# evergreen-ci/evergreen

Hardware: NVIDIA H100
Metric: tasks scheduled/sec over N distros; host-allocator decisions/sec at 1/2/4/8 GPU (higher is better)
Workload: dtype int64

## Files before the change

evergreen_b200/csrc/evg_plan_general.cuh:

```cuda
#pragma once

#ifndef EVG_OCC_GLINK
#define EVG_OCC_GLINK 4
#endif
#ifndef EVG_OCC_GALLOC
#define EVG_OCC_GALLOC 4
#endif
#ifndef EVG_OCC_GFILL
#define EVG_OCC_GFILL 4
#endif
#ifndef EVG_OCC_GUNIT
#define EVG_OCC_GUNIT 4
#endif
#ifndef EVG_OCC_GBEST
#define EVG_OCC_GBEST 4
#endif
#ifndef EVG_GTASK_OCC
#define EVG_GTASK_OCC 2
#endif
constexpr int kGTile = 2048;

struct DGen {
  int64_t n_tiles;
  int64_t tile0;
  const int32_t* tile_distro;
  const int64_t* tile_start;
  const int64_t* dtile_off;
  unsigned long long* vmm;
  uint32_t* key_lo[2];
  uint32_t* key_hi[2];
  uint32_t* idx[2];
  uint32_t* e;
  uint32_t* tile_sum;
  uint32_t* tile_hist;
  uint4* wl;
  struct URec* pay;
  unsigned int* ccount;
  uint4* tie;
  int32_t* maxpass;
  uint32_t* run;
  uint32_t* pown;
  uint32_t* pver;
  uint32_t* pedge;
  uint32_t* sedge;
  uint32_t* rank;
  unsigned int* rcount;
  uint2* blist;
  unsigned int* bcount;
  uint4* usum;
  uint2* hlist;
  unsigned int* hcount;
  int64_t* tv;
};

__device__ __forceinline__ int gen_bits(const DGen& G, int d) {
  const unsigned long long r = G.vmm[2 * d] - G.vmm[2 * d + 1];
  return r == 0 ? 0 : 64 - __clzll((long long)r);
}
__device__ __forceinline__ int gen_npass(int bits) { return (bits + 7) >> 3; }

struct __align__(16) URec {
  int32_t prio, nd;
  int64_t exp_ns, qb;
  int32_t tgo;
  uint32_t lif;
};
static_assert(sizeof(URec) == 32, "one L2 sector per member");
constexpr uint32_t kRecGrouped = 1u << 22, kRecWaitOver = 1u << 23;
constexpr uint32_t kRunOwn = 1u << 31, kRunEntry = kRunOwn - 1u;
__device__ __forceinline__ uint32_t rec_li(const URec& r) { return r.lif & 0x1FFFFFu; }
__device__ __forceinline__ URec rec_load(const URec* p) {
  const uint4 a = reinterpret_cast<const uint4*>(p)[0], b = reinterpret_cast<const uint4*>(p)[1];
  URec r;
  r.prio = int32_t(a.x); r.nd = int32_t(a.y); r.exp_ns = int64_t((unsigned long long)a.z | ((unsigned long long)a.w << 32));
  r.qb = int64_t((unsigned long long)b.x | ((unsigned long long)b.y << 32)); r.tgo = int32_t(b.z); r.lif = b.w;
  return r;
}
__device__ __forceinline__ void rec_store(URec* p, const URec& r) {
  reinterpret_cast<uint4*>(p)[0] = make_uint4(uint32_t(r.prio), uint32_t(r.nd), uint32_t(uint64_t(r.exp_ns)), uint32_t(uint64_t(r.exp_ns) >> 32));
  reinterpret_cast<uint4*>(p)[1] = make_uint4(uint32_t(uint64_t(r.qb)), uint32_t(uint64_t(r.qb) >> 32), uint32_t(r.tgo), r.lif);
}

__global__ void k_ginit(DGen G, const int32_t* __restrict__ general_list, int n) {
  const int k = blockIdx.x * blockDim.x + threadIdx.x;
  if (k == 0) { *G.ccount = 0u; *G.maxpass = 0; *G.rcount = 0u; *G.hcount = 0u; *G.bcount = 0u; }
  if (k >= n) return;
  const int d = general_list[k];
  G.vmm[2 * d] = 0ull;
  G.vmm[2 * d + 1] = ~0ull;
}

__global__ void __launch_bounds__(256) k_gmark(DTasks T, DDistros D, DWork W, DGen G) {
  if (*W.err) return;
  const int tile = int(blockIdx.x + G.tile0);
  const int d = G.tile_distro[tile];
  const int64_t base = D.task_off[d], end = D.task_off[d + 1];
  const int64_t lo = max(G.tile_start[tile], base), hi = min(G.tile_start[tile] + kGTile, end);
  for (int64_t t = lo + threadIdx.x; t < hi; t += 256)
    for (int64_t e = T.dep_off[t]; e < T.dep_off[t + 1]; e++) W.has_dep[base + T.dep_idx[e]] = 1;
}

struct TileFold {
  unsigned int c[10];
  unsigned long long s[4];
// ... 478 lines not shown
      }
      if (lane == 0) {
        if (hi > __ldcg(G.vmm + 2 * d0)) atomicMax(G.vmm + 2 * d0, hi);
        if (lo < __ldcg(G.vmm + 2 * d0 + 1)) atomicMin(G.vmm + 2 * d0 + 1, lo);
      }
    } else if (d >= 0) {
      if (kk > __ldcg(G.vmm + 2 * d)) atomicMax(G.vmm + 2 * d, kk);
      if (kk < __ldcg(G.vmm + 2 * d + 1)) atomicMin(G.vmm + 2 * d + 1, kk);
    }
  }
}

__global__ void k_gsched(DGen G, const int32_t* __restrict__ general_list, int n) {
  const int k = blockIdx.x * blockDim.x + threadIdx.x;
  if (k >= n) return;
  const int np = gen_npass(gen_bits(G, general_list[k]));
  if (np > 0) atomicMax(G.maxpass, np);
}

__global__ void __launch_bounds__(256) k_gsum(DDistros D, DGen G) {
  const int tile = int(blockIdx.x + G.tile0);
  const int d = G.tile_distro[tile];
  const int64_t base = D.task_off[d], end = D.task_off[d + 1];
  const int64_t lo = max(G.tile_start[tile], base), hi = min(G.tile_start[tile] + kGTile, end);
  uint32_t sum = 0;
  for (int64_t t = lo + threadIdx.x; t < hi; t += 256) sum += G.e[t];
  sum = __reduce_add_sync(0xffffffffu, sum);
  __shared__ uint32_t sw[8];
  if ((threadIdx.x & 31) == 0) sw[threadIdx.x >> 5] = sum;
  __syncthreads();
  if (threadIdx.x == 0) G.tile_sum[tile] = sw[0] + sw[1] + sw[2] + sw[3] + sw[4] + sw[5] + sw[6] + sw[7];
}
// ... 32 lines not shown

__device__ __forceinline__ void gen_put(const DGen& G, int64_t base, uint32_t pos, unsigned long long vmax_ord, bool wide,
                                        int64_t v, uint32_t li) {
  const unsigned long long key = vmax_ord - ord_i64(v);
  G.key_lo[0][base + pos] = uint32_t(key);
  if (wide) G.key_hi[0][base + pos] = uint32_t(key >> 32);
  G.idx[0][base + pos] = li;
}

__global__ void __launch_bounds__(256) k_gplace(DDistros D, DWork W, DGen G, int use_e) {
  const int tile = int(blockIdx.x + G.tile0);
  const int d = G.tile_distro[tile];
  const int64_t base = D.task_off[d], end = D.task_off[d + 1];
  const int64_t ts = G.tile_start[tile];
  const unsigned long long vmax_ord = G.vmm[2 * d];
  const bool wide = gen_bits(G, d) > 32;
  const int tid = threadIdx.x, lane = tid & 31, warp = tid >> 5;
  const int64_t t8 = ts + 8 * int64_t(tid);
  const bool interior = t8 >= base && t8 + 7 < end;
  uint32_t ev[8];
  uint32_t sum = 0;
  if (use_e) {
    if (interior) {
      const uint4 a = *reinterpret_cast<const uint4*>(G.e + t8), b = *reinterpret_cast<const uint4*>(G.e + t8 + 4);
      ev[0] = a.x; ev[1] = a.y; ev[2] = a.z; ev[3] = a.w; ev[4] = b.x; ev[5] = b.y; ev[6] = b.z; ev[7] = b.w;
    } else {
#pragma unroll
      for (int m = 0; m < 8; m++) { const int64_t t = t8 + m; ev[m] = (t >= base && t < end) ? G.e[t] : 0u; }
    }
#pragma unroll
    for (int m = 0; m < 8; m++) sum += ev[m];
// ... 20 lines not shown
      vv[m] = x.x; vv[m + 1] = x.y;
    }
    if (use_e) {
      const uint32_t h0 = *reinterpret_cast<const uint32_t*>(W.has_dep + t8), h1 = *reinterpret_cast<const uint32_t*>(W.has_dep + t8 + 4);
#pragma unroll
      for (int m = 0; m < 4; m++) dsp |= (((h0 >> (8 * m + 1)) & 1u) << m) | (((h1 >> (8 * m + 1)) & 1u) << (m + 4));
    }
  } else {
#pragma unroll
    for (int m = 0; m < 8; m++) {
      const int64_t t = t8 + m;
      const bool in = t >= base && t < end;
      vv[m] = in ? G.tv[t] : 0;
      if (use_e && in && (W.has_dep[t] & 2)) dsp |= 1u << m;
    }
  }
  if (use_e) {
    constexpr int kStage = 3072;
    __shared__ uint32_t st_lo[kStage], st_ix[kStage], st_hi[kStage];
    __shared__ uint32_t s_total;
    const uint32_t p_tile = G.tile_sum[tile];
    if (tid == 255) s_total = run + sum - p_tile;
    uint32_t ps[8];
#pragma unroll
    for (int m = 0; m < 8; m++) { ps[m] = run; run += ev[m]; }
    if (interior) {
      *reinterpret_cast<uint4*>(G.e + t8) = make_uint4(ps[0], ps[1], ps[2], ps[3]);
      *reinterpret_cast<uint4*>(G.e + t8 + 4) = make_uint4(ps[4], ps[5], ps[6], ps[7]);
    } else {
#pragma unroll
// ... 64 lines not shown
  uint32_t pos = G.e[base + a];
  const uint32_t cnt = W.unit_n[slot];
  if (cnt <= 64) {
    pos += __popcll(W.unit_mask[slot] & ((1ull << myrk) - 1ull));
  } else {
    const uint32_t* run = G.run + W.head[slot];
    for (uint32_t i = 0; i < cnt; i++) {
      const uint4 tq = G.tie[run[i] & kRunEntry];
      if (tq.z == slot && tq.y < myrk) pos++;
    }
  }
  gen_put(G, base, pos, G.vmm[2 * d], gen_bits(G, d) > 32, G.tv[t], uint32_t(int64_t(t) - base));
  }
}

__device__ __forceinline__ bool gen_tile(const DDistros& D, const DGen& G, int tile, int j, int* d_out, int64_t* seg, int64_t* lo,
                                         int* cnt, bool* wide) {
  const int d = G.tile_distro[tile];
  const int bits = gen_bits(G, d);
  if (j >= gen_npass(bits)) return false;
  const int64_t base = D.task_off[d], end = D.task_off[d + 1];
  const int64_t a = max(G.tile_start[tile], base), b = min(G.tile_start[tile] + kGTile, end);
  *d_out = d; *seg = base; *lo = a; *cnt = int(b - a); *wide = bits > 32;
  return true;
}

__global__ void __launch_bounds__(256) k_ghist(int j, DDistros D, DGen G) {
  if (j >= *G.maxpass) return;
  int d, cnt; int64_t seg, lo; bool wide;
  const int tile = int(blockIdx.x + G.tile0);
  if (!gen_tile(D, G, tile, j, &d, &seg, &lo, &cnt, &wide)) return;
  const uint32_t* src = (j < 4 ? G.key_lo[j & 1] : G.key_hi[j & 1]) + lo;
  const int shift = 8 * (j & 3);
  __shared__ uint32_t h[256];
  h[threadIdx.x] = 0;
  __syncthreads();
  for (int i = threadIdx.x; i < cnt; i += 256) atomicAdd(&h[(src[i] >> shift) & 255u], 1u);
  __syncthreads();
  G.tile_hist[int64_t(tile) * 256 + threadIdx.x] = h[threadIdx.x];
}

__global__ void __launch_bounds__(1024) k_gdscan(int j, const int32_t* __restrict__ general_list, DGen G) {
  if (j >= *G.maxpass) return;
  const int d = general_list[blockIdx.x];
  if (j >= gen_npass(gen_bits(G, d))) return;
  const int dg = threadIdx.x & 255, grp = threadIdx.x >> 8;
  const int64_t t0 = G.dtile_off[d], nt = G.dtile_off[d + 1] - t0;
  const int64_t per = (nt + 3) / 4;
  const int64_t a = t0 + (grp * per < nt ? grp * per : nt), b = t0 + ((grp + 1) * per < nt ? (grp + 1) * per : nt);
  uint32_t* h = G.tile_hist + dg;
  uint32_t sum = 0;
  int64_t tile = a;
  for (; tile + 8 <= b; tile += 8) {
    uint32_t x[8];
#pragma unroll
    for (int k = 0; k < 8; k++) x[k] = h[(tile + k) * 256];
#pragma unroll
    for (int k = 0; k < 8; k++) sum += x[k];
  }
  for (; tile < b; tile++) sum += h[tile * 256];
  __shared__ uint32_t part[4][256];
  __shared__ uint32_t s[256];
  part[grp][dg] = sum;
  __syncthreads();
  const uint32_t total = part[0][dg] + part[1][dg] + part[2][dg] + part[3][dg];
  if (grp == 0) s[dg] = total;
  __syncthreads();
  for (int o = 1; o < 256; o <<= 1) {
    uint32_t v = 0;
    if (grp == 0 && dg >= o) v = s[dg - o];
    __syncthreads();
    if (grp == 0) s[dg] += v;
    __syncthreads();
  }
  uint32_t run = s[dg] - total;
  for (int g = 0; g < grp; g++) run += part[g][dg];
  tile = a;
  for (; tile + 8 <= b; tile += 8) {
    uint32_t x[8];
#pragma unroll
    for (int k = 0; k < 8; k++) x[k] = h[(tile + k) * 256];
#pragma unroll
    for (int k = 0; k < 8; k++) { h[(tile + k) * 256] = run; run += x[k]; }
  }
  for (; tile < b; tile++) { const uint32_t x = h[tile * 256]; h[tile * 256] = run; run += x; }
}

template <bool WIDE>
__device__ __forceinline__ void gscatter_tile(int j, const DGen& G, int tile, int64_t seg, int64_t lo, int cnt, uint32_t (*wcnt)[256],
                                              uint32_t* s_lo, uint32_t* s_ix, uint32_t* s_hi, int32_t* s_delta, uint32_t* s_wsum) {
  constexpr bool wide = WIDE;
  const int sb = j & 1, db = sb ^ 1;
  const int tid = threadIdx.x, warp = tid >> 5, lane = tid & 31;
#pragma unroll
  for (int w = 0; w < 8; w++) wcnt[w][tid] = 0u;
  __syncthreads();
  const unsigned lt = (1u << lane) - 1u;
  const int shift = 8 * (j & 3);
  const bool use_hi = j >= 4;
  const uint32_t* src_lo = G.key_lo[sb] + lo;
  const uint32_t* src_hi = G.key_hi[sb] + lo;
  const uint32_t* src_ix = G.idx[sb] + lo;
  uint32_t kl[8], kh[8], ix[8], dg[8], rk[8];
#pragma unroll
  for (int k = 0; k < 8; k++) {
    const int i = (warp * 8 + k) * 32 + lane;
    const bool ok = i < cnt;
    kl[k] = ok ? src_lo[i] : 0u;
    kh[k] = (ok && wide) ? src_hi[i] : 0u;
    ix[k] = ok ? src_ix[i] : 0u;
  }
  unsigned peers[8];
#pragma unroll
  for (int k = 0; k < 8; k++) {
    const int i = (warp * 8 + k) * 32 + lane;
    dg[k] = i < cnt ? (((use_hi ? kh[k] : kl[k]) >> shift) & 255u) : 256u;
    peers[k] = __match_any_sync(0xffffffffu, dg[k]);
  }
#pragma unroll
  for (int k = 0; k < 8; k++) {
    rk[k] = 0;
    if (dg[k] < 256u && (peers[k] & lt) == 0u) rk[k] = atomicAdd(&wcnt[warp][dg[k]], uint32_t(__popc(peers[k])));
  }
#pragma unroll
  for (int k = 0; k < 8; k++) rk[k] = __shfl_sync(0xffffffffu, rk[k], __ffs(peers[k]) - 1) + uint32_t(__popc(peers[k] & lt));
  __syncthreads();
  {
    uint32_t x[8], tot = 0;
#pragma unroll
    for (int w = 0; w < 8; w++) { x[w] = wcnt[w][tid]; tot += x[w]; }
    uint32_t inc = tot;
#pragma unroll
    for (int o = 1; o < 32; o <<= 1) { const uint32_t y = __shfl_up_sync(0xffffffffu, inc, o); if (lane >= o) inc += y; }
    if (lane == 31) s_wsum[warp] = inc;
    __syncthreads();
    uint32_t before = 0;
#pragma unroll
    for (int w = 0; w < 8; w++) before += w < warp ? s_wsum[w] : 0u;
    const uint32_t lbase = before + inc - tot;
    s_delta[tid] = int32_t(G.tile_hist[int64_t(tile) * 256 + tid]) - int32_t(lbase);
    uint32_t run = lbase;
#pragma unroll
    for (int w = 0; w < 8; w++) { wcnt[w][tid] = run; run += x[w]; }
  }
  __syncthreads();
#pragma unroll
  for (int k = 0; k < 8; k++) {
    if (dg[k] < 256u) {
      const uint32_t lp = wcnt[warp][dg[k]] + rk[k];
      s_lo[lp] = kl[k];
      s_ix[lp] = ix[k];
      if (wide) s_hi[lp] = kh[k];
    }
  }
  __syncthreads();
  uint32_t* dst_lo = G.key_lo[db] + seg;
  uint32_t* dst_hi = G.key_hi[db] + seg;
  uint32_t* dst_ix = G.idx[db] + seg;
  for (int i = tid; i < cnt; i += 256) {
    const uint32_t a = s_lo[i], h = wide ? s_hi[i] : 0u;
    const uint32_t dgt = ((use_hi ? h : a) >> shift) & 255u;
    const int64_t pos = int64_t(s_delta[dgt]) + i;
    dst_lo[pos] = a;
    dst_ix[pos] = s_ix[i];
    if (wide) dst_hi[pos] = h;
  }
}

__global__ void __launch_bounds__(256, 4) k_gscatter(int j, DDistros D, DGen G) {
  if (j >= *G.maxpass) return;
  int d, cnt; int64_t seg, lo; bool wide;
  const int tile = int(blockIdx.x + G.tile0);
  if (!gen_tile(D, G, tile, j, &d, &seg, &lo, &cnt, &wide)) return;
  __shared__ uint32_t wcnt[8][256];
  __shared__ uint32_t s_lo[kGTile], s_ix[kGTile], s_hi[kGTile];
  __shared__ int32_t s_delta[256];
  __shared__ uint32_t s_wsum[8];
  if (wide) gscatter_tile<true>(j, G, tile, seg, lo, cnt, wcnt, s_lo, s_ix, s_hi, s_delta, s_wsum);
  else gscatter_tile<false>(j, G, tile, seg, lo, cnt, wcnt, s_lo, s_ix, s_hi, s_delta, s_wsum);
}

__global__ void __launch_bounds__(256) k_gemit(DDistros D, DGen G, int32_t* __restrict__ order, int64_t* __restrict__ total_value) {
  const int tile = int(blockIdx.x + G.tile0);
  const int d = G.tile_distro[tile];
  const int64_t base = D.task_off[d], end = D.task_off[d + 1];
  const int64_t lo = max(G.tile_start[tile], base), hi = min(G.tile_start[tile] + kGTile, end);
  const int bits = gen_bits(G, d);
  const int fin = gen_npass(bits) & 1;
  const bool wide = bits > 32;
  const unsigned long long vmax_ord = G.vmm[2 * d];
  for (int64_t p = lo + threadIdx.x; p < hi; p += 256) {
    unsigned long long key = G.key_lo[fin][p];
    if (wide) key |= (unsigned long long)G.key_hi[fin][p] << 32;
    order[p] = int32_t(G.idx[fin][p]);
    total_value[p] = unord_i64(vmax_ord - key);
  }
}
```

evergreen_b200/csrc/evg_sched.cu:

```cuda
#include <cuda_runtime.h>
#include <stdarg.h>
#include <stdint.h>
#include <stdio.h>
#include <string.h>

#include <algorithm>
#include <type_traits>
#include <cstdlib>
#include <future>
#include <mutex>
#include <string>
#include <vector>

#include "evg_score.cuh"
#include "evg_intern.h"

using namespace evg;

namespace {

thread_local std::string g_err;

int fail(int code, const char* fmt, ...) {
  char buf[512];
// ... 1093 lines not shown
  } dp;
  DevBuf b_err;
  DevBuf b_route, b_unitv, b_unita, b_unitn, b_unitmask;
  DevBuf b_punt, b_puntcnt;
  struct RouteList {
    std::vector<int32_t> h;
    DevBuf b, lpt;
    int32_t n() const { return int32_t(h.size()); }
  };
  RouteList routes[kRoutes];
  int64_t max_cta_tasks = 0;
  int32_t nNA_big = 0;
  DevBuf b_alist;
  int64_t n_alist = 0;
  bool alist_valid = false;
  std::vector<int64_t> h_taskoff, h_groupoff, h_unitbase, h_edgeoff, h_dtileoff;
  std::vector<int32_t> h_nver;
  cudaStream_t s_h2d = nullptr, s_d2h = nullptr;
  static constexpr int kMaxChunks = 16;
  cudaEvent_t ev_h[kMaxChunks] = {}, ev_c[kMaxChunks] = {};
  int general_complex = 0;
  int64_t Tgc = 0;
  DevBuf b_kv, b_vmm, b_klo[2], b_khi[2], b_ix[2], b_e, b_tilesum, b_gmisc;
  DevBuf b_tiledistro, b_tilestart, b_dtileoff, b_tilehist, b_wl, b_pay, b_place, b_eplace, b_run, b_rank, b_blist, b_tie, b_hlist, b_usum, b_upd;
  DevBuf b_qinfo, b_ginfo, b_order, b_tv, b_bd;
  DevBuf b_hflags, b_hgid, b_hexp, b_hstd, b_hstart, b_hostoff, b_acfg, b_gs, b_result, b_status;
  bool bd_valid = false;
  evg_alloc_result* ext_result = nullptr;
  int64_t ext_capacity = 0;
  evg_alloc_result* result_ptr() const { return ext_result ? ext_result : b_result.as<evg_alloc_result>(); }
};

namespace {

DTasks dtasks(const evg_ctx* c);
DDistros ddistros(const evg_ctx* c);
DWork dwork(const evg_ctx* c);
DGen dgen(const evg_ctx* c);
inline unsigned grid_for(int64_t n, int block) { return unsigned((n + block - 1) / block); }
// ... 27 lines not shown
                 const int64_t* edge_off = nullptr) {
  const bool copy_columns = cols == Cols::kCopy, adopt = cols == Cols::kAdopt;
  if (!t || !dt) return fail(EVG_ERR_INVALID, "null task table / distro table");
  const int64_t T = t->n_tasks, E = t->n_edges;
  const int32_t D = dt->n_distros;
  if (T < 0 || E < 0 || D < 0) return fail(EVG_ERR_INVALID, "negative sizes");
  if (T >= (int64_t(1) << 31) - 2) return fail(EVG_ERR_INVALID, "n_tasks %lld exceeds 2^31-2 per call", (long long)T);
  if (2 * T + E >= int64_t(0xFFFFFFF0u)) return fail(EVG_ERR_INVALID, "2*n_tasks+n_edges exceeds the 32-bit pair id space");
  if (D > 0 && (!dt->task_off || !dt->group_off || !dt->cfg)) return fail(EVG_ERR_INVALID, "null distro arrays");
  if (T > 0 && task_cols_missing(t)) return fail(EVG_ERR_INVALID, "null task column");
  if (E > 0 && (!t->dep_off || !t->dep_idx)) return fail(EVG_ERR_INVALID, "n_edges > 0 but dep_off/dep_idx null");
  if (D == 0 && T != 0) return fail(EVG_ERR_INVALID, "tasks without distros");
  int rc = D > 0 ? check_offsets(dt->task_off, D, T, who, "task_off") : EVG_OK;
  if (rc == EVG_OK && D > 0) rc = check_offsets(dt->group_off, D, -1, who, "group_off");
  if (rc != EVG_OK) return rc;
  std::vector<int64_t> unit_base(size_t(D) + 1, 0), dtile_off(size_t(D) + 1, 0);
  std::vector<int32_t> tile_distro, list[kRoutes];
  std::vector<int64_t> tile_start;
  std::vector<uint8_t> route(size_t(D) + 1, 0);
  int general_complex = 0;
  int any_complex = E > 0 ? 1 : 0;
  int64_t Tgc = 0, Prec = 0;
  constexpr int kGA = PlanCta<kNT_A, kNCapA>::kGroupCap, kGB = PlanCta<kNT_B, kNCapB>::kGroupCap, kGC = PlanCta<kNT_C, kNCapC>::kGroupCap;
  constexpr int kBigUnits = kRoutes;
  auto size_class = [&](int32_t d) -> int {
    const int64_t a = dt->task_off[d], b = dt->task_off[d + 1];
    const int64_t n = b - a, g = dt->group_off[d + 1] - dt->group_off[d];
    const evg_distro_cfg& cf = dt->cfg[d];
    const int64_t de = (E > 0) ? (edge_off ? edge_off[d + 1] - edge_off[d] : t->dep_off[b] - t->dep_off[a]) : 0;
    const bool narrow = !cf.group_versions && de == 0;
    if (n <= kCapW) return kWarp;
    if (narrow && n <= kNCapA && g <= kGA) return kCtaA;
// ... 22 lines not shown
    if (gb > ga || cf.group_versions) any_complex = 1;
    unit_base[d + 1] = unit_base[d] + (gb - ga) + (cf.group_versions ? int64_t(cf.n_versions) : (b - a));
    const int64_t n = b - a;
    const int64_t de = (E > 0) ? (edge_off ? edge_off[d + 1] - edge_off[d] : t->dep_off[b] - t->dep_off[a]) : 0;
    const int r = route_of(d);
    list[r].push_back(d);
    route[d] = r != kGeneral;
    if (r == kGeneral) {
      if (gb > ga || cf.group_versions || de > 0) {
        general_complex = 1;
        Tgc += n;
        Prec += n + ((cf.group_versions && gb > ga) ? n : 0) + de;
      }
      const int64_t a0 = a & ~int64_t(3);
      for (int64_t s = a0; s < b; s += kGTile) { tile_distro.push_back(d); tile_start.push_back(s); }
    }
    dtile_off[d + 1] = int64_t(tile_distro.size());
  }
  const int64_t G = D > 0 ? dt->group_off[D] : 0;
  if (G > 0 && !dt->group_max_hosts) return fail(EVG_ERR_INVALID, "null group_max_hosts");
  const int64_t U = unit_base[D];
  if (U >= int64_t(0xFFFFFFF0u)) return fail(EVG_ERR_INVALID, "unit slot space exceeds 32 bits");
  if (Prec >= int64_t(0xFFFFFFF0u)) return fail(EVG_ERR_INVALID, "unit table exceeds 32 bits");
  if (Tgc >= int64_t(kRunOwn)) return fail(EVG_ERR_INVALID, "work list exceeds 31 bits (a run position is entry id | own bit)");
  const int64_t NT = int64_t(tile_distro.size());
  const int64_t P = 2 * T + E;
  cudaStream_t s = c->stream;
  drop_tick(c);
#define UPC(buf, ptr, count, type)                                                                    \
  do {                                                                                                \
    if (cols == Cols::kResident) break;                                                               \
    if (adopt) {                                                                                      \
      if ((reinterpret_cast<uintptr_t>(ptr) & 15u) != 0) return fail(EVG_ERR_INVALID, "device column %s is not 16-byte aligned", #ptr); \
      (buf).adopt(const_cast<void*>(static_cast<const void*>(ptr)));                                  \
    } else {                                                                                          \
      CK((buf).ensure(sizeof(type) * size_t((count) + kColPad)));                                     \
      if (copy_columns && (count) > 0) CK(cudaMemcpyAsync((buf).p, (ptr), sizeof(type) * size_t(count), cudaMemcpyHostToDevice, s)); \
    }                                                                                                 \
  } while (0)
  UPC(c->tasks.prio, t->priority, T, int32_t);
// ... 6 lines not shown
  UPC(c->tasks.vid, t->version_id, T, int32_t);
  UPC(c->tasks.flags, t->flags, T, uint32_t);
  if (E > 0) {
    UPC(c->b_depoff, t->dep_off, T + 1, int64_t);
    UPC(c->b_depidx, t->dep_idx, E, int32_t);
  }
#undef UPC
  UP(s, c->b_taskoff, dt->task_off, D + 1, int64_t);
  UP(s, c->b_groupoff, dt->group_off, D + 1, int64_t);
  UP(s, c->b_cfg, dt->cfg, D, evg_distro_cfg);
  UP(s, c->b_gmax, dt->group_max_hosts, G, int32_t);
  UP(s, c->b_unitbase, unit_base.data(), D + 1, int64_t);
  UP(s, c->b_tiledistro, tile_distro.data(), NT, int32_t);
  UP(s, c->b_tilestart, tile_start.data(), NT, int64_t);
  UP(s, c->b_dtileoff, dtile_off.data(), D + 1, int64_t);
  UP(s, c->b_route, route.data(), D + 1, uint8_t);
  for (int r = 0; r < kRoutes; r++) UP(s, c->routes[r].b, list[r].data(), int64_t(list[r].size()), int32_t);
  std::vector<int32_t> lpt[kRoutes];
  for (int r = 0; r < kRoutes; r++) {
    if (!largest_first(r)) continue;
    lpt[r] = list[r];
    std::stable_sort(lpt[r].begin(), lpt[r].end(), [&](int32_t x, int32_t y) {
      return dt->task_off[x + 1] - dt->task_off[x] > dt->task_off[y + 1] - dt->task_off[y];
    });
  }
  constexpr int kGS = PlanCta<kNT_S, kNCapS>::kGroupCap;
  auto fits_s = [&](int32_t x) { return dt->task_off[x + 1] - dt->task_off[x] <= kNCapS && dt->group_off[x + 1] - dt->group_off[x] <= kGS; };
  std::vector<int32_t>& lpt_a = lpt[kCtaA];
  std::stable_partition(lpt_a.begin(), lpt_a.end(), [&](int32_t x) { return !fits_s(x); });
  c->nNA_big = int32_t(std::count_if(lpt_a.begin(), lpt_a.end(), [&](int32_t x) { return !fits_s(x); }));
// ... 18 lines not shown
    CK(c->b_unita.ensure(sizeof(uint32_t) * size_t(U + 1)));
    CK(c->b_unitn.ensure(sizeof(uint32_t) * size_t(U + 1)));
    CK(c->b_unitmask.ensure(sizeof(uint64_t) * size_t(U + 1)));
    CK(c->b_bestpair.ensure(sizeof(uint32_t) * size_t(T + 1)));
  }
  if (on_chip) CK(c->b_kv.ensure(sizeof(uint64_t) * size_t(T + 1)));
  if (!list[kGeneral].empty()) {
    for (int k = 0; k < 2; k++) {
      CK(c->b_klo[k].ensure(sizeof(uint32_t) * size_t(T + 1)));
      CK(c->b_khi[k].ensure(sizeof(uint32_t) * size_t(T + 1)));
      CK(c->b_ix[k].ensure(sizeof(uint32_t) * size_t(T + 1)));
    }
    CK(c->b_vmm.ensure(sizeof(uint64_t) * 2 * size_t(D + 1)));
    CK(c->b_gmisc.ensure(64));
    CK(c->b_tilesum.ensure(sizeof(uint32_t) * size_t(NT + 1)));
    CK(c->b_tilehist.ensure(sizeof(uint32_t) * 256 * size_t(NT + 1)));
    if (general_complex) {
      CK(c->b_e.ensure(sizeof(uint32_t) * size_t(T + kColPad)));
      CK(c->b_wl.ensure(sizeof(uint4) * size_t(Tgc + 1)));
      CK(c->b_pay.ensure(sizeof(URec) * size_t(Tgc + 1)));
      CK(c->b_tie.ensure(sizeof(uint4) * size_t(Tgc + 1)));
      CK(c->b_place.ensure(sizeof(uint32_t) * 2 * size_t(Tgc + 1)));
      CK(c->b_eplace.ensure(sizeof(uint32_t) * 2 * size_t(E + 1)));
      CK(c->b_run.ensure(sizeof(uint32_t) * size_t(Prec + 1)));
      CK(c->b_rank.ensure(sizeof(uint32_t) * size_t(Prec + 1)));
      CK(c->b_blist.ensure(sizeof(uint2) * size_t(Prec / kRankOne + 1)));
      CK(c->b_hlist.ensure(sizeof(uint2) * size_t(Prec + 1)));
      CK(c->b_usum.ensure(sizeof(uint4) * size_t(U + 1)));
    }
  }
  CK(c->b_punt.ensure(sizeof(int32_t) * size_t(D + 1)));
// ... 9 lines not shown
  for (int32_t d = 0; d < D; d++) c->max_groups = std::max(c->max_groups, dt->group_off[d + 1] - dt->group_off[d]);
  c->any_complex = any_complex;
  c->general_complex = general_complex;
  CK(c->b_err.ensure(sizeof(int) * 4));
  CK(cudaMemsetAsync(c->b_err.p, 0, sizeof(int) * 4, s));
  for (int r = 0; r < kRoutes; r++) c->routes[r].h.swap(list[r]);
  c->h_taskoff.assign(dt->task_off, dt->task_off + D + 1);
  c->h_groupoff.assign(dt->group_off, dt->group_off + D + 1);
  c->h_edgeoff.assign(size_t(D) + 1, 0);
  if (E > 0)
    for (int32_t d = 0; d <= D; d++) c->h_edgeoff[size_t(d)] = edge_off ? edge_off[d] : t->dep_off[dt->task_off[d]];
  c->h_nver.resize(size_t(D));
  for (int32_t d = 0; d < D; d++) c->h_nver[size_t(d)] = dt->cfg[d].n_versions;
  c->h_unitbase.swap(unit_base);
  c->h_dtileoff.swap(dtile_off);
  c->tick.kind = adopt ? Tick::kBorrowed : Tick::kFixed;
  c->alist_valid = false;
  if (cols != Cols::kChunked && T > 0) {
    DTasks dtv = dtasks(c);
    DDistros ddv = ddistros(c);
    DWork wv = dwork(c);
    k_validate<<<grid_for(T, 256), 256, 0, s>>>(dtv, ddv, wv, 0, T);
    int bad = 0;
    CK(cudaMemcpyAsync(&bad, c->b_err.p, sizeof(int), cudaMemcpyDeviceToHost, s));
    CK(cudaStreamSynchronize(s));
    if (bad) { drop_tick(c); return fail(EVG_ERR_INVALID, "a group_id / version_id / dep_idx is out of range for its distro"); }
  }
  return EVG_OK;
}

// ... 54 lines not shown
  w.best_pair = c->b_bestpair.as<uint32_t>();
  w.buf[0].key_v = c->b_kv.as<uint64_t>();
  w.qinfo = c->b_qinfo.as<evg_queue_info>(); w.ginfo = c->b_ginfo.as<evg_group_info>();
  return w;
}
DGen dgen(const evg_ctx* c) {
  DGen g;
  g.n_tiles = c->NT;
  g.tile0 = 0;
  g.tile_distro = c->b_tiledistro.as<int32_t>(); g.tile_start = c->b_tilestart.as<int64_t>();
  g.dtile_off = c->b_dtileoff.as<int64_t>();
  g.vmm = c->b_vmm.as<unsigned long long>();
  for (int k = 0; k < 2; k++) {
    g.key_lo[k] = c->b_klo[k].as<uint32_t>(); g.key_hi[k] = c->b_khi[k].as<uint32_t>(); g.idx[k] = c->b_ix[k].as<uint32_t>();
  }
  g.e = c->b_e.as<uint32_t>(); g.tile_sum = c->b_tilesum.as<uint32_t>(); g.tile_hist = c->b_tilehist.as<uint32_t>();
  g.wl = c->b_wl.as<uint4>();
  g.pay = c->b_pay.as<URec>();
  g.pown = c->b_place.as<uint32_t>();
  g.pver = c->b_place.as<uint32_t>() + (c->Tgc + 1);
  g.pedge = c->b_eplace.as<uint32_t>();
  g.sedge = c->b_eplace.as<uint32_t>() + (c->E + 1);
  g.ccount = c->b_gmisc.as<unsigned int>();
  g.maxpass = c->b_gmisc.as<int32_t>() + 1;
  g.rcount = c->b_gmisc.as<unsigned int>() + 2;
  g.hcount = c->b_gmisc.as<unsigned int>() + 3;
  g.bcount = c->b_gmisc.as<unsigned int>() + 4;
  g.blist = c->b_blist.as<uint2>();
  g.rank = c->b_rank.as<uint32_t>();
  g.hlist = c->b_hlist.as<uint2>();
  g.usum = c->b_usum.as<uint4>();
// ... 82 lines not shown
    CK(cudaMemsetAsync(c->b_unitn.as<uint32_t>() + u0, 0, sizeof(uint32_t) * size_t(u1 - u0), s));
  }
  return EVG_OK;
}

int run_general(evg_ctx* c, cudaStream_t st, const DTasks& dt, const DDistros& dd, const DWork& w, int64_t now, int32_t gfirst,
                int32_t gcount) {
  if (gcount <= 0) return EVG_OK;
  DGen g = dgen(c);
  const int gc = c->general_complex;
  const std::vector<int32_t>& gh = c->routes[kGeneral].h;
  const int32_t d_first = gh[size_t(gfirst)], d_last = gh[size_t(gfirst + gcount - 1)];
  g.tile0 = c->h_dtileoff[size_t(d_first)];
  const unsigned nt = unsigned(c->h_dtileoff[size_t(d_last) + 1] - g.tile0);
  const int32_t* gl = c->routes[kGeneral].b.as<int32_t>() + gfirst;
  LAUNCH_ON(c, st, k_ginit, grid_for(gcount, 256), 256, g, gl, gcount);
  if (gc && c->E > 0) LAUNCH_ON(c, st, k_gmark, nt, 256, dt, dd, w, g);
  if (c->timed) CK(cudaEventRecord(c->ev_gt0, st));
  LAUNCH_ON(c, st, k_gtask, nt, 256, dt, dd, w, g, now, gc);
  if (c->timed) { CK(cudaEventRecord(c->ev_gt1, st)); c->general_timed = true; }
  const unsigned wl_grid = unsigned(std::min<int64_t>(std::max<int64_t>(1, (c->Tgc + 255) / 256), int64_t(c->num_sms) * 16));
  if (gc) {
    LAUNCH_ON(c, st, k_glink, wl_grid, 256, dt, dd, w, g, now);
    LAUNCH_ON(c, st, k_galloc, wl_grid, 256, dt, dd, w, g);
    LAUNCH_ON(c, st, k_gfill, wl_grid, 256, dt, dd, w, g);
    LAUNCH_ON(c, st, k_gunit, wl_grid, 256, dd, w, g, now);
    LAUNCH_ON(c, st, k_grank, wl_grid, 256, w, g);
    LAUNCH_ON(c, st, k_gbest, wl_grid, 256, dt, dd, w, g, c->bd_valid ? 1 : 0);
  }
  LAUNCH_ON(c, st, k_gsched, grid_for(gcount, 128), 128, g, gl, gcount);
  if (gc) {
    LAUNCH_ON(c, st, k_gsum, nt, 256, dd, g);
    LAUNCH_ON(c, st, k_gscan, unsigned(gcount), 1024, g, gl);
  }
  LAUNCH_ON(c, st, k_gplace, nt, 256, dd, w, g, gc);
  if (gc) LAUNCH_ON(c, st, k_gplace_disp, wl_grid, 256, dt, dd, w, g);
  if (c->timed) CK(cudaEventRecord(c->ev_sort0, st));
  for (int j = 0; j < 8; j++) {
    LAUNCH_ON(c, st, k_ghist, nt, 256, j, dd, g);
    LAUNCH_ON(c, st, k_gdscan, unsigned(gcount), 1024, j, gl, g);
    LAUNCH_ON(c, st, k_gscatter, nt, 256, j, dd, g);
  }
  if (c->timed) CK(cudaEventRecord(c->ev_sort1, st));
  LAUNCH_ON(c, st, k_gemit, nt, 256, dd, g, c->b_order.as<int32_t>(), c->b_tv.as<int64_t>());
  const int64_t g0 = c->h_groupoff[size_t(d_first)], g1 = c->h_groupoff[size_t(d_last) + 1];
  LAUNCH_ON(c, st, k_finalize_info, grid_for(std::max<int64_t>(d_last + 1 - d_first, g1 - g0), 256), 256, dd, w, d_first, d_last + 1, g0, g1);
  return EVG_OK;
}

int ensure_aux_streams(evg_ctx* c) {
  if (c->ev_fork) return EVG_OK;
  for (int k = 0; k < evg_ctx::kAux; k++) {
    CK(cudaStreamCreateWithFlags(&c->s_aux[k], cudaStreamNonBlocking));
    CK(cudaEventCreateWithFlags(&c->ev_join[k], cudaEventDisableTiming));
  }
  CK(cudaEventCreateWithFlags(&c->ev_fork, cudaEventDisableTiming));
  return EVG_OK;
}

// ... 2269 lines not shown
```

Measured before the change: 4.510 billion.

## Replace per-pass hist/scan/scatter radix sort with one-sweep decoupled lookback sort

Builds all eight digit histograms per distro once during placement and drops the per-pass tile histogram and distro scan kernels. Each radix pass now becomes a single persistent scatter kernel that takes tiles by atomic ticket and resolves offsets with decoupled lookback over epoch-tagged status words. The final pass writes order and total values directly, which removes the emit kernel, and sort tiles double in size. This cuts launches and global histogram traffic, at the cost of spin-waiting, a bounded-poll failure path and extra shared memory per block.

After: 4.645 billion (median of 6 runs). 1.03x the previous value.

```diff
diff --git a/evergreen_b200/csrc/evg_plan_general.cuh b/evergreen_b200/csrc/evg_plan_general.cuh
--- a/evergreen_b200/csrc/evg_plan_general.cuh
+++ b/evergreen_b200/csrc/evg_plan_general.cuh
@@ -32,7 +32,12 @@
   uint32_t* idx[2];
   uint32_t* e;
   uint32_t* tile_sum;
-  uint32_t* tile_hist;
+  const int32_t* stile;
+  int64_t stile0;
+  uint32_t* status;
+  uint32_t* dhist;
+  int32_t* gpos;
+  unsigned int* ticket;
   uint4* wl;
   struct URec* pay;
   unsigned int* ccount;
@@ -57,7 +62,7 @@
   const unsigned long long r = G.vmm[2 * d] - G.vmm[2 * d + 1];
   return r == 0 ? 0 : 64 - __clzll((long long)r);
 }
-__device__ __forceinline__ int gen_npass(int bits) { return (bits + 7) >> 3; }
+__device__ __forceinline__ int gen_npass(int bits) { return max(1, (bits + 7) >> 3); }
 
 struct __align__(16) URec {
   int32_t prio, nd;
@@ -81,13 +86,18 @@
   reinterpret_cast<uint4*>(p)[1] = make_uint4(uint32_t(uint64_t(r.qb)), uint32_t(uint64_t(r.qb) >> 32), uint32_t(r.tgo), r.lif);
 }
 
-__global__ void k_ginit(DGen G, const int32_t* __restrict__ general_list, int n) {
-  const int k = blockIdx.x * blockDim.x + threadIdx.x;
-  if (k == 0) { *G.ccount = 0u; *G.maxpass = 0; *G.rcount = 0u; *G.hcount = 0u; *G.bcount = 0u; }
+__global__ void k_ginit(DGen G, const int32_t* __restrict__ general_list, int n, int gfirst) {
+  const int64_t k = int64_t(blockIdx.x) * blockDim.x + threadIdx.x;
+  if (k == 0) {
+    *G.ccount = 0u; *G.maxpass = 0; *G.rcount = 0u; *G.hcount = 0u; *G.bcount = 0u;
+    for (int j = 0; j < 8; j++) G.ticket[j] = 0u;
+  }
+  if (k < int64_t(n) * 512) reinterpret_cast<uint4*>(G.dhist + int64_t(gfirst) * 2048)[k] = make_uint4(0u, 0u, 0u, 0u);
   if (k >= n) return;
   const int d = general_list[k];
   G.vmm[2 * d] = 0ull;
   G.vmm[2 * d + 1] = ~0ull;
+  G.gpos[d] = gfirst + int(k);
 }
 
 __global__ void __launch_bounds__(256) k_gmark(DTasks T, DDistros D, DWork W, DGen G) {
@@ -596,8 +606,7 @@
 __global__ void k_gsched(DGen G, const int32_t* __restrict__ general_list, int n) {
   const int k = blockIdx.x * blockDim.x + threadIdx.x;
   if (k >= n) return;
-  const int np = gen_npass(gen_bits(G, general_list[k]));
-  if (np > 0) atomicMax(G.maxpass, np);
+  atomicMax(G.maxpass, gen_npass(gen_bits(G, general_list[k])));
 }
 
 __global__ void __launch_bounds__(256) k_gsum(DDistros D, DGen G) {
@@ -660,7 +669,8 @@
   const int64_t base = D.task_off[d], end = D.task_off[d + 1];
   const int64_t ts = G.tile_start[tile];
   const unsigned long long vmax_ord = G.vmm[2 * d];
-  const bool wide = gen_bits(G, d) > 32;
+  const int bits = gen_bits(G, d);
+  const bool wide = bits > 32;
   const int tid = threadIdx.x, lane = tid & 31, warp = tid >> 5;
   const int64_t t8 = ts + 8 * int64_t(tid);
   const bool interior = t8 >= base && t8 + 7 < end;
@@ -711,6 +721,24 @@
       vv[m] = in ? G.tv[t] : 0;
       if (use_e && in && (W.has_dep[t] & 2)) dsp |= 1u << m;
     }
+  }
+  {
+    __shared__ uint32_t s_h[8][256];
+    const int np = gen_npass(bits);
+    for (int j = 0; j < np; j++) s_h[j][tid] = 0u;
+    __syncthreads();
+#pragma unroll
+    for (int m = 0; m < 8; m++) {
+      const int64_t t = t8 + m;
+      if (t >= base && t < end) {
+        const unsigned long long key = vmax_ord - ord_i64(vv[m]);
+        for (int j = 0; j < np; j++) atomicAdd(&s_h[j][uint32_t(key >> (8 * j)) & 255u], 1u);
+      }
+    }
+    __syncthreads();
+    uint32_t* dh = G.dhist + int64_t(G.gpos[d]) * 2048 + tid;
+    for (int j = 0; j < np; j++)
+      if (s_h[j][tid]) atomicAdd(dh + 256 * j, s_h[j][tid]);
   }
   if (use_e) {
     constexpr int kStage = 3072;
@@ -805,86 +833,44 @@
   }
 }
 
-__device__ __forceinline__ bool gen_tile(const DDistros& D, const DGen& G, int tile, int j, int* d_out, int64_t* seg, int64_t* lo,
-                                         int* cnt, bool* wide) {
-  const int d = G.tile_distro[tile];
-  const int bits = gen_bits(G, d);
-  if (j >= gen_npass(bits)) return false;
-  const int64_t base = D.task_off[d], end = D.task_off[d + 1];
-  const int64_t a = max(G.tile_start[tile], base), b = min(G.tile_start[tile] + kGTile, end);
-  *d_out = d; *seg = base; *lo = a; *cnt = int(b - a); *wide = bits > 32;
-  return true;
-}
-
-__global__ void __launch_bounds__(256) k_ghist(int j, DDistros D, DGen G) {
-  if (j >= *G.maxpass) return;
-  int d, cnt; int64_t seg, lo; bool wide;
-  const int tile = int(blockIdx.x + G.tile0);
-  if (!gen_tile(D, G, tile, j, &d, &seg, &lo, &cnt, &wide)) return;
-  const uint32_t* src = (j < 4 ? G.key_lo[j & 1] : G.key_hi[j & 1]) + lo;
-  const int shift = 8 * (j & 3);
-  __shared__ uint32_t h[256];
-  h[threadIdx.x] = 0;
-  __syncthreads();
-  for (int i = threadIdx.x; i < cnt; i += 256) atomicAdd(&h[(src[i] >> shift) & 255u], 1u);
-  __syncthreads();
-  G.tile_hist[int64_t(tile) * 256 + threadIdx.x] = h[threadIdx.x];
-}
-
-__global__ void __launch_bounds__(1024) k_gdscan(int j, const int32_t* __restrict__ general_list, DGen G) {
-  if (j >= *G.maxpass) return;
-  const int d = general_list[blockIdx.x];
-  if (j >= gen_npass(gen_bits(G, d))) return;
-  const int dg = threadIdx.x & 255, grp = threadIdx.x >> 8;
-  const int64_t t0 = G.dtile_off[d], nt = G.dtile_off[d + 1] - t0;
-  const int64_t per = (nt + 3) / 4;
-  const int64_t a = t0 + (grp * per < nt ? grp * per : nt), b = t0 + ((grp + 1) * per < nt ? (grp + 1) * per : nt);
-  uint32_t* h = G.tile_hist + dg;
-  uint32_t sum = 0;
-  int64_t tile = a;
-  for (; tile + 8 <= b; tile += 8) {
-    uint32_t x[8];
-#pragma unroll
-    for (int k = 0; k < 8; k++) x[k] = h[(tile + k) * 256];
-#pragma unroll
-    for (int k = 0; k < 8; k++) sum += x[k];
-  }
-  for (; tile < b; tile++) sum += h[tile * 256];
-  __shared__ uint32_t part[4][256];
-  __shared__ uint32_t s[256];
-  part[grp][dg] = sum;
-  __syncthreads();
-  const uint32_t total = part[0][dg] + part[1][dg] + part[2][dg] + part[3][dg];
-  if (grp == 0) s[dg] = total;
-  __syncthreads();
-  for (int o = 1; o < 256; o <<= 1) {
-    uint32_t v = 0;
-    if (grp == 0 && dg >= o) v = s[dg - o];
-    __syncthreads();
-    if (grp == 0) s[dg] += v;
-    __syncthreads();
-  }
-  uint32_t run = s[dg] - total;
-  for (int g = 0; g < grp; g++) run += part[g][dg];
-  tile = a;
-  for (; tile + 8 <= b; tile += 8) {
-    uint32_t x[8];
-#pragma unroll
-    for (int k = 0; k < 8; k++) x[k] = h[(tile + k) * 256];
-#pragma unroll
-    for (int k = 0; k < 8; k++) { h[(tile + k) * 256] = run; run += x[k]; }
-  }
-  for (; tile < b; tile++) { const uint32_t x = h[tile * 256]; h[tile * 256] = run; run += x; }
-}
+constexpr int kSortTiles = 2;
+constexpr int kSortN = kSortTiles * kGTile;
+constexpr int kSortThreads = 256 * kSortTiles;
+constexpr int kSortWarps = kSortThreads / 32;
+static_assert(kMaxTasksPerDistro < (int64_t(1) << 21), "a status word holds a position inside a distro in 21 bits");
+
+constexpr uint32_t kStInclusive = 1u << 21, kStCount = kStInclusive - 1u;
+constexpr int kStEpochShift = 22;
+constexpr uint32_t kGenEpochs = 1u << (32 - kStEpochShift);
+constexpr unsigned kSpinPolls = 1u << 22;
+__device__ __forceinline__ uint32_t gen_status_load(const uint32_t* p) {
+  uint32_t v;
+  asm volatile("ld.relaxed.gpu.global.u32 %0, [%1];" : "=r"(v) : "l"(p) : "memory");
+  return v;
+}
+__device__ __forceinline__ void gen_status_store(uint32_t* p, uint32_t v) {
+  asm volatile("st.relaxed.gpu.global.u32 [%0], %1;" ::"l"(p), "r"(v) : "memory");
+}
+constexpr int kLookWindow = 4;
+
+struct GSortSmem {
+  uint32_t wcnt[kSortWarps][256];
+  uint32_t lo[kSortN], ix[kSortN], hi[kSortN];
+  int32_t delta[256];
+  uint32_t wsum[8], hsum[8];
+  uint32_t tile;
+  int bad;
+};
 
 template <bool WIDE>
-__device__ __forceinline__ void gscatter_tile(int j, const DGen& G, int tile, int64_t seg, int64_t lo, int cnt, uint32_t (*wcnt)[256],
-                                              uint32_t* s_lo, uint32_t* s_ix, uint32_t* s_hi, int32_t* s_delta, uint32_t* s_wsum) {
+__device__ __forceinline__ void gscatter_tile(int j, uint32_t epoch, const DGen& G, int64_t st, int d, bool first, bool last,
+                                              int64_t seg, int64_t lo, int cnt, GSortSmem& S, int* err,
+                                              int32_t* __restrict__ order, int64_t* __restrict__ total_value) {
   constexpr bool wide = WIDE;
   const int sb = j & 1, db = sb ^ 1;
   const int tid = threadIdx.x, warp = tid >> 5, lane = tid & 31;
-#pragma unroll
-  for (int w = 0; w < 8; w++) wcnt[w][tid] = 0u;
+  for (int i = tid; i < kSortWarps * 256; i += kSortThreads) (&S.wcnt[0][0])[i] = 0u;
+  if (tid == 0) S.bad = 0;
   __syncthreads();
   const unsigned lt = (1u << lane) - 1u;
   const int shift = 8 * (j & 3);
@@ -911,79 +897,123 @@
 #pragma unroll
   for (int k = 0; k < 8; k++) {
     rk[k] = 0;
-    if (dg[k] < 256u && (peers[k] & lt) == 0u) rk[k] = atomicAdd(&wcnt[warp][dg[k]], uint32_t(__popc(peers[k])));
+    if (dg[k] < 256u && (peers[k] & lt) == 0u) rk[k] = atomicAdd(&S.wcnt[warp][dg[k]], uint32_t(__popc(peers[k])));
   }
 #pragma unroll
   for (int k = 0; k < 8; k++) rk[k] = __shfl_sync(0xffffffffu, rk[k], __ffs(peers[k]) - 1) + uint32_t(__popc(peers[k] & lt));
   __syncthreads();
-  {
-    uint32_t x[8], tot = 0;
-#pragma unroll
-    for (int w = 0; w < 8; w++) { x[w] = wcnt[w][tid]; tot += x[w]; }
-    uint32_t inc = tot;
-#pragma unroll
-    for (int o = 1; o < 32; o <<= 1) { const uint32_t y = __shfl_up_sync(0xffffffffu, inc, o); if (lane >= o) inc += y; }
-    if (lane == 31) s_wsum[warp] = inc;
-    __syncthreads();
-    uint32_t before = 0;
-#pragma unroll
-    for (int w = 0; w < 8; w++) before += w < warp ? s_wsum[w] : 0u;
-    const uint32_t lbase = before + inc - tot;
-    s_delta[tid] = int32_t(G.tile_hist[int64_t(tile) * 256 + tid]) - int32_t(lbase);
+  uint32_t tot = 0, inc = 0, h = 0, hinc = 0;
+  if (tid < 256) {
+    for (int w = 0; w < kSortWarps; w++) tot += S.wcnt[w][tid];
+    if (first) h = G.dhist[(int64_t(G.gpos[d]) * 8 + j) * 256 + tid];
+    inc = tot; hinc = h;
+#pragma unroll
+    for (int o = 1; o < 32; o <<= 1) {
+      const uint32_t y = __shfl_up_sync(0xffffffffu, inc, o), z = __shfl_up_sync(0xffffffffu, hinc, o);
+      if (lane >= o) { inc += y; hinc += z; }
+    }
+    if (lane == 31) { S.wsum[warp] = inc; S.hsum[warp] = hinc; }
+  }
+  __syncthreads();
+  uint32_t lbase = 0, excl = 0;
+  uint32_t* sw = G.status + st * 256 + tid;
+  const uint32_t tag = epoch << kStEpochShift;
+  if (tid < 256) {
+    uint32_t before = 0, hbefore = 0;
+#pragma unroll
+    for (int w = 0; w < 8; w++) { before += w < warp ? S.wsum[w] : 0u; hbefore += w < warp ? S.hsum[w] : 0u; }
+    lbase = before + inc - tot;
+    excl = hbefore + hinc - h;
+    gen_status_store(sw, tag | (first ? kStInclusive | (excl + tot) : tot));
     uint32_t run = lbase;
-#pragma unroll
-    for (int w = 0; w < 8; w++) { wcnt[w][tid] = run; run += x[w]; }
+    for (int w = 0; w < kSortWarps; w++) { const uint32_t x = S.wcnt[w][tid]; S.wcnt[w][tid] = run; run += x; }
   }
   __syncthreads();
 #pragma unroll
   for (int k = 0; k < 8; k++) {
     if (dg[k] < 256u) {
-      const uint32_t lp = wcnt[warp][dg[k]] + rk[k];
-      s_lo[lp] = kl[k];
-      s_ix[lp] = ix[k];
-      if (wide) s_hi[lp] = kh[k];
-    }
+      const uint32_t lp = S.wcnt[warp][dg[k]] + rk[k];
+      S.lo[lp] = kl[k];
+      S.ix[lp] = ix[k];
+      if (wide) S.hi[lp] = kh[k];
+    }
+  }
+  if (tid < 256) {
+    if (!first) {
+      excl = 0;
+      int64_t p = st - 1;
+      unsigned polls = 0;
+      for (bool done = false; !done;) {
+        uint32_t w[kLookWindow];
+#pragma unroll
+        for (int k = 0; k < kLookWindow; k++) w[k] = p >= k ? gen_status_load(G.status + (p - k) * 256 + tid) : 0u;
+        bool stall = false;
+#pragma unroll
+        for (int k = 0; k < kLookWindow; k++) {
+          if (done || stall) continue;
+          if ((w[k] >> kStEpochShift) != epoch) { stall = true; continue; }
+          excl += w[k] & kStCount;
+          done = (w[k] & kStInclusive) != 0;
+          p--;
+        }
+        if (stall) {
+          if (++polls == kSpinPolls) { S.bad = 1; break; }
+          if (polls > 32) __nanosleep(min(32u << min(polls - 32u, 5u), 1024u));
+        }
+      }
+      gen_status_store(sw, tag | kStInclusive | (excl + tot));
+    }
+    S.delta[tid] = int32_t(excl) - int32_t(lbase);
   }
   __syncthreads();
+  if (S.bad) {
+    if (tid == 0) atomicOr(err, 2);
+    return;
+  }
+  if (last) {
+    const unsigned long long vmax_ord = G.vmm[2 * d];
+    for (int i = tid; i < cnt; i += kSortThreads) {
+      const uint32_t a = S.lo[i], hw = wide ? S.hi[i] : 0u;
+      const int64_t pos = seg + int64_t(S.delta[((use_hi ? hw : a) >> shift) & 255u]) + i;
+      order[pos] = int32_t(S.ix[i]);
+      total_value[pos] = unord_i64(vmax_ord - ((unsigned long long)hw << 32 | a));
+    }
+    return;
+  }
   uint32_t* dst_lo = G.key_lo[db] + seg;
   uint32_t* dst_hi = G.key_hi[db] + seg;
   uint32_t* dst_ix = G.idx[db] + seg;
-  for (int i = tid; i < cnt; i += 256) {
-    const uint32_t a = s_lo[i], h = wide ? s_hi[i] : 0u;
-    const uint32_t dgt = ((use_hi ? h : a) >> shift) & 255u;
-    const int64_t pos = int64_t(s_delta[dgt]) + i;
+  for (int i = tid; i < cnt; i += kSortThreads) {
+    const uint32_t a = S.lo[i], hw = wide ? S.hi[i] : 0u;
+    const int64_t pos = int64_t(S.delta[((use_hi ? hw : a) >> shift) & 255u]) + i;
     dst_lo[pos] = a;
-    dst_ix[pos] = s_ix[i];
-    if (wide) dst_hi[pos] = h;
-  }
-}
-
-__global__ void __launch_bounds__(256, 4) k_gscatter(int j, DDistros D, DGen G) {
-  if (j >= *G.maxpass) return;
-  int d, cnt; int64_t seg, lo; bool wide;
-  const int tile = int(blockIdx.x + G.tile0);
-  if (!gen_tile(D, G, tile, j, &d, &seg, &lo, &cnt, &wide)) return;
-  __shared__ uint32_t wcnt[8][256];
-  __shared__ uint32_t s_lo[kGTile], s_ix[kGTile], s_hi[kGTile];
-  __shared__ int32_t s_delta[256];
-  __shared__ uint32_t s_wsum[8];
-  if (wide) gscatter_tile<true>(j, G, tile, seg, lo, cnt, wcnt, s_lo, s_ix, s_hi, s_delta, s_wsum);
-  else gscatter_tile<false>(j, G, tile, seg, lo, cnt, wcnt, s_lo, s_ix, s_hi, s_delta, s_wsum);
-}
-
-__global__ void __launch_bounds__(256) k_gemit(DDistros D, DGen G, int32_t* __restrict__ order, int64_t* __restrict__ total_value) {
-  const int tile = int(blockIdx.x + G.tile0);
-  const int d = G.tile_distro[tile];
-  const int64_t base = D.task_off[d], end = D.task_off[d + 1];
-  const int64_t lo = max(G.tile_start[tile], base), hi = min(G.tile_start[tile] + kGTile, end);
-  const int bits = gen_bits(G, d);
-  const int fin = gen_npass(bits) & 1;
-  const bool wide = bits > 32;
-  const unsigned long long vmax_ord = G.vmm[2 * d];
-  for (int64_t p = lo + threadIdx.x; p < hi; p += 256) {
-    unsigned long long key = G.key_lo[fin][p];
-    if (wide) key |= (unsigned long long)G.key_hi[fin][p] << 32;
-    order[p] = int32_t(G.idx[fin][p]);
-    total_value[p] = unord_i64(vmax_ord - key);
-  }
-}
+    dst_ix[pos] = S.ix[i];
+    if (wide) dst_hi[pos] = hw;
+  }
+}
+
+__global__ void __launch_bounds__(kSortThreads, 4 / kSortTiles) k_gscatter(int j, uint32_t epoch, unsigned nst, DDistros D, DGen G,
+                                                                           int* err, int32_t* __restrict__ order,
+                                                                           int64_t* __restrict__ total_value) {
+  if (j >= *G.maxpass || *err) return;
+  extern __shared__ __align__(16) unsigned char gs_smem[];
+  GSortSmem& S = *reinterpret_cast<GSortSmem*>(gs_smem);
+  for (;;) {
+    __syncthreads();
+    if (threadIdx.x == 0) S.tile = atomicAdd(G.ticket + j, 1u);
+    __syncthreads();
+    if (S.tile >= nst) return;
+    const int64_t st = G.stile0 + S.tile;
+    const int tile = G.stile[st];
+    const int d = G.tile_distro[tile];
+    const int bits = gen_bits(G, d);
+    const int np = gen_npass(bits);
+    if (j >= np) continue;
+    const int64_t base = D.task_off[d], end = D.task_off[d + 1];
+    const int64_t lo = max(G.tile_start[tile], base), hi = min(G.tile_start[tile] + kSortN, end);
+    const bool first = tile == G.dtile_off[d], last = j == np - 1;
+    if (bits > 32) gscatter_tile<true>(j, epoch, G, st, d, first, last, base, lo, int(hi - lo), S, err, order, total_value);
+    else gscatter_tile<false>(j, epoch, G, st, d, first, last, base, lo, int(hi - lo), S, err, order, total_value);
+    if (S.bad) return;
+  }
+}
diff --git a/evergreen_b200/csrc/evg_sched.cu b/evergreen_b200/csrc/evg_sched.cu
--- a/evergreen_b200/csrc/evg_sched.cu
+++ b/evergreen_b200/csrc/evg_sched.cu
@@ -1131,7 +1131,8 @@
   DevBuf b_alist;
   int64_t n_alist = 0;
   bool alist_valid = false;
-  std::vector<int64_t> h_taskoff, h_groupoff, h_unitbase, h_edgeoff, h_dtileoff;
+  std::vector<int64_t> h_taskoff, h_groupoff, h_unitbase, h_edgeoff, h_dtileoff, h_dstileoff;
+  uint32_t gen_epoch = 0;
   std::vector<int32_t> h_nver;
   cudaStream_t s_h2d = nullptr, s_d2h = nullptr;
   static constexpr int kMaxChunks = 16;
@@ -1139,7 +1140,7 @@
   int general_complex = 0;
   int64_t Tgc = 0;
   DevBuf b_kv, b_vmm, b_klo[2], b_khi[2], b_ix[2], b_e, b_tilesum, b_gmisc;
-  DevBuf b_tiledistro, b_tilestart, b_dtileoff, b_tilehist, b_wl, b_pay, b_place, b_eplace, b_run, b_rank, b_blist, b_tie, b_hlist, b_usum, b_upd;
+  DevBuf b_tiledistro, b_tilestart, b_dtileoff, b_stile, b_lookback, b_dhist, b_gpos, b_wl, b_pay, b_place, b_eplace, b_run, b_rank, b_blist, b_tie, b_hlist, b_usum, b_upd;
   DevBuf b_qinfo, b_ginfo, b_order, b_tv, b_bd;
   DevBuf b_hflags, b_hgid, b_hexp, b_hstd, b_hstart, b_hostoff, b_acfg, b_gs, b_result, b_status;
   bool bd_valid = false;
@@ -1197,8 +1198,8 @@
   int rc = D > 0 ? check_offsets(dt->task_off, D, T, who, "task_off") : EVG_OK;
   if (rc == EVG_OK && D > 0) rc = check_offsets(dt->group_off, D, -1, who, "group_off");
   if (rc != EVG_OK) return rc;
-  std::vector<int64_t> unit_base(size_t(D) + 1, 0), dtile_off(size_t(D) + 1, 0);
-  std::vector<int32_t> tile_distro, list[kRoutes];
+  std::vector<int64_t> unit_base(size_t(D) + 1, 0), dtile_off(size_t(D) + 1, 0), dstile_off(size_t(D) + 1, 0);
+  std::vector<int32_t> tile_distro, stile, list[kRoutes];
   std::vector<int64_t> tile_start;
   std::vector<uint8_t> route(size_t(D) + 1, 0);
   int general_complex = 0;
@@ -1251,8 +1252,10 @@
       }
       const int64_t a0 = a & ~int64_t(3);
       for (int64_t s = a0; s < b; s += kGTile) { tile_distro.push_back(d); tile_start.push_back(s); }
+      for (int64_t k = dtile_off[d]; k < int64_t(tile_distro.size()); k += kSortTiles) stile.push_back(int32_t(k));
     }
     dtile_off[d + 1] = int64_t(tile_distro.size());
+    dstile_off[d + 1] = int64_t(stile.size());
   }
   const int64_t G = D > 0 ? dt->group_off[D] : 0;
   if (G > 0 && !dt->group_max_hosts) return fail(EVG_ERR_INVALID, "null group_max_hosts");
@@ -1260,7 +1263,7 @@
   if (U >= int64_t(0xFFFFFFF0u)) return fail(EVG_ERR_INVALID, "unit slot space exceeds 32 bits");
   if (Prec >= int64_t(0xFFFFFFF0u)) return fail(EVG_ERR_INVALID, "unit table exceeds 32 bits");
   if (Tgc >= int64_t(kRunOwn)) return fail(EVG_ERR_INVALID, "work list exceeds 31 bits (a run position is entry id | own bit)");
-  const int64_t NT = int64_t(tile_distro.size());
+  const int64_t NT = int64_t(tile_distro.size()), NST = int64_t(stile.size());
   const int64_t P = 2 * T + E;
   cudaStream_t s = c->stream;
   drop_tick(c);
@@ -1297,6 +1300,7 @@
   UP(s, c->b_tiledistro, tile_distro.data(), NT, int32_t);
   UP(s, c->b_tilestart, tile_start.data(), NT, int64_t);
   UP(s, c->b_dtileoff, dtile_off.data(), D + 1, int64_t);
+  UP(s, c->b_stile, stile.data(), NST, int32_t);
   UP(s, c->b_route, route.data(), D + 1, uint8_t);
   for (int r = 0; r < kRoutes; r++) UP(s, c->routes[r].b, list[r].data(), int64_t(list[r].size()), int32_t);
   std::vector<int32_t> lpt[kRoutes];
@@ -1345,7 +1349,9 @@
     CK(c->b_vmm.ensure(sizeof(uint64_t) * 2 * size_t(D + 1)));
     CK(c->b_gmisc.ensure(64));
     CK(c->b_tilesum.ensure(sizeof(uint32_t) * size_t(NT + 1)));
-    CK(c->b_tilehist.ensure(sizeof(uint32_t) * 256 * size_t(NT + 1)));
+    CK(c->b_lookback.ensure(sizeof(uint32_t) * 256 * size_t(NST + 1)));
+    CK(c->b_dhist.ensure(sizeof(uint32_t) * 2048 * list[kGeneral].size()));
+    CK(c->b_gpos.ensure(sizeof(int32_t) * size_t(D + 1)));
     if (general_complex) {
       CK(c->b_e.ensure(sizeof(uint32_t) * size_t(T + kColPad)));
       CK(c->b_wl.ensure(sizeof(uint4) * size_t(Tgc + 1)));
@@ -1385,6 +1391,8 @@
   for (int32_t d = 0; d < D; d++) c->h_nver[size_t(d)] = dt->cfg[d].n_versions;
   c->h_unitbase.swap(unit_base);
   c->h_dtileoff.swap(dtile_off);
+  c->h_dstileoff.swap(dstile_off);
+  c->gen_epoch = 0;
   c->tick.kind = adopt ? Tick::kBorrowed : Tick::kFixed;
   c->alist_valid = false;
   if (cols != Cols::kChunked && T > 0) {
@@ -1469,7 +1477,10 @@
   for (int k = 0; k < 2; k++) {
     g.key_lo[k] = c->b_klo[k].as<uint32_t>(); g.key_hi[k] = c->b_khi[k].as<uint32_t>(); g.idx[k] = c->b_ix[k].as<uint32_t>();
   }
-  g.e = c->b_e.as<uint32_t>(); g.tile_sum = c->b_tilesum.as<uint32_t>(); g.tile_hist = c->b_tilehist.as<uint32_t>();
+  g.e = c->b_e.as<uint32_t>(); g.tile_sum = c->b_tilesum.as<uint32_t>();
+  g.stile = c->b_stile.as<int32_t>(); g.stile0 = 0;
+  g.status = c->b_lookback.as<uint32_t>(); g.dhist = c->b_dhist.as<uint32_t>(); g.gpos = c->b_gpos.as<int32_t>();
+  g.ticket = c->b_gmisc.as<unsigned int>() + 8;
   g.wl = c->b_wl.as<uint4>();
   g.pay = c->b_pay.as<URec>();
   g.pown = c->b_place.as<uint32_t>();
@@ -1582,7 +1593,7 @@
   g.tile0 = c->h_dtileoff[size_t(d_first)];
   const unsigned nt = unsigned(c->h_dtileoff[size_t(d_last) + 1] - g.tile0);
   const int32_t* gl = c->routes[kGeneral].b.as<int32_t>() + gfirst;
-  LAUNCH_ON(c, st, k_ginit, grid_for(gcount, 256), 256, g, gl, gcount);
+  LAUNCH_ON(c, st, k_ginit, grid_for(int64_t(gcount) * 512, 256), 256, g, gl, gcount, gfirst);
   if (gc && c->E > 0) LAUNCH_ON(c, st, k_gmark, nt, 256, dt, dd, w, g);
   if (c->timed) CK(cudaEventRecord(c->ev_gt0, st));
   LAUNCH_ON(c, st, k_gtask, nt, 256, dt, dd, w, g, now, gc);
@@ -1603,14 +1614,26 @@
   }
   LAUNCH_ON(c, st, k_gplace, nt, 256, dd, w, g, gc);
   if (gc) LAUNCH_ON(c, st, k_gplace_disp, wl_grid, 256, dt, dd, w, g);
+  if (c->gen_epoch == 0 || c->gen_epoch + 16 > kGenEpochs) {
+    CK(cudaMemsetAsync(c->b_lookback.p, 0, sizeof(uint32_t) * 256 * size_t(c->h_dstileoff.back() + 1), st));
+    c->gen_epoch = 0;
+  }
+  c->gen_epoch += 8;
+  g.stile0 = c->h_dstileoff[size_t(d_first)];
+  const unsigned nst = unsigned(c->h_dstileoff[size_t(d_last) + 1] - g.stile0);
+  CK(cudaFuncSetAttribute(k_gscatter, cudaFuncAttributeMaxDynamicSharedMemorySize, int(sizeof(GSortSmem))));
+  int per_sm = 0;
+  CK(cudaOccupancyMaxActiveBlocksPerMultiprocessor(&per_sm, k_gscatter, kSortThreads, sizeof(GSortSmem)));
+  const unsigned sgrid = unsigned(std::min<int64_t>(nst, int64_t(std::max(per_sm, 1)) * c->num_sms));
   if (c->timed) CK(cudaEventRecord(c->ev_sort0, st));
   for (int j = 0; j < 8; j++) {
-    LAUNCH_ON(c, st, k_ghist, nt, 256, j, dd, g);
-    LAUNCH_ON(c, st, k_gdscan, unsigned(gcount), 1024, j, gl, g);
-    LAUNCH_ON(c, st, k_gscatter, nt, 256, j, dd, g);
+    if (nst > 0) {
+      k_gscatter<<<sgrid, kSortThreads, sizeof(GSortSmem), st>>>(j, c->gen_epoch + uint32_t(j), nst, dd, g, w.err,
+                                                                c->b_order.as<int32_t>(), c->b_tv.as<int64_t>());
+      c->launches++;
+    }
   }
   if (c->timed) CK(cudaEventRecord(c->ev_sort1, st));
-  LAUNCH_ON(c, st, k_gemit, nt, 256, dd, g, c->b_order.as<int32_t>(), c->b_tv.as<int64_t>());
   const int64_t g0 = c->h_groupoff[size_t(d_first)], g1 = c->h_groupoff[size_t(d_last) + 1];
   LAUNCH_ON(c, st, k_finalize_info, grid_for(std::max<int64_t>(d_last + 1 - d_first, g1 - g0), 256), 256, dd, w, d_first, d_last + 1, g0, g1);
   return EVG_OK;
```
